# thu-ml/stochastic_gcn

Hardware: AMD Instinct MI355X
Metric: training edges/s (SpMM) (higher is better)
Workload: dtype f32

## Files before the change

stochastic_gcn_amd/csrc/sgcn_dense.hip:

```cpp
#include <algorithm>

#include "sgcn_dev.h"
#include "sgcn_fuse.h"

namespace sgcn {

__device__ __forceinline__ float wave_sum(float v) {
#pragma unroll
    for (int o = 32; o > 0; o >>= 1) v += __shfl_xor(v, o, 64);
    return v;
}
__device__ __forceinline__ float wave_max(float v) {
#pragma unroll
    for (int o = 32; o > 0; o >>= 1) v = fmaxf(v, __shfl_xor(v, o, 64));
    return v;
}

__global__ __launch_bounds__(kBlock) void ln_act_fwd_kernel(
    const float* __restrict__ x, int64_t ldx, const float* __restrict__ offset,
    const float* __restrict__ scale, int32_t n, int32_t d, float eps, int32_t norm, int32_t relu,
    float* __restrict__ y, int64_t ldy, float* __restrict__ xhat, float* __restrict__ rstd) {
    const int lane = threadIdx.x & 63;
    const int64_t row = (int64_t)blockIdx.x * (kBlock / kWave) + threadIdx.x / kWave;
    if (row >= n) return;
// ... 7 lines not shown
    for (int c = lane; c < d; c += kWave) s += xr[c];
    const float mean = wave_sum(s) / (float)d;
    float q = 0.f;
    for (int c = lane; c < d; c += kWave) { const float t = xr[c] - mean; q += t * t; }
    const float r = rsqrtf(wave_sum(q) / (float)d + eps);
    if (lane == 0) rstd[row] = r;
    float* hr = xhat + row * (int64_t)d;
    for (int c = lane; c < d; c += kWave) {
        const float h = (xr[c] - mean) * r;
        hr[c] = h;
        const float v = h * scale[c] + offset[c];
        yr[c] = relu ? fmaxf(v, 0.f) : v;
    }
}

struct LnBwdDx { const float* W; int32_t K, kg; DropArgs drop; float* dxo; int64_t lddxo;
                 int32_t dma; };
struct LnBwdNext { const float* y; int64_t ldy; const float* xhat; const float* rstd; const float* scale; int32_t norm, relu;
                   float* g; float* partial; };

__device__ __forceinline__ void ln_bwd_stats(float g, float h, float sc, float& doff, float& dsc, float& s1, float& s2) {
#pragma clang fp contract(off)
    doff += g;
    dsc = fmaf(g, h, dsc);
    const float t2 = g * sc;
    s1 += t2;
    s2 = fmaf(t2, h, s2);
}
__device__ __forceinline__ float ln_bwd_out(float g, float h, float sc, float m1, float m2, float r) {
#pragma clang fp contract(off)
    return r * fmaf(-h, m2, fmaf(g, sc, -m1));
}

constexpr int kBwdRowsPerWave = 1;
__global__ __launch_bounds__(kBlock) void ln_act_bwd_kernel(
    const float* __restrict__ dy, int64_t lddy, const float* __restrict__ y, int64_t ldy,
    const float* __restrict__ xhat, const float* __restrict__ rstd, const float* __restrict__ scale,
    int32_t n, int32_t d, int32_t norm, int32_t relu, float* __restrict__ dx, int64_t lddx,
    float* __restrict__ partial , LnBwdDx t, LnBwdNext nx) {
    extern __shared__ float lds[];
    const int lane = threadIdx.x & 63, wave = threadIdx.x / kWave;
    const int64_t row0 = ((int64_t)blockIdx.x * (kBlock / kWave) + wave) * kBwdRowsPerWave;
    float* my = lds + (size_t)wave * 2 * d;
    float* wt = lds + (norm ? (size_t)8 * d : 0);
    const int kp = t.K + 1;
    const int wregion = t.dma ? (t.K * d + 255) / 256 * 256 : d * kp;
    if (t.W && t.dma) {
        const int P = d >> 2, sh = __ffs(P) - 1, total4 = t.K * P;
        for (int base4 = wave * kWave; base4 < total4; base4 += kBlock) {
            const int sl = min(base4 + lane, total4 - 1);
            const int j = sl >> sh, src4 = (j << sh) + ((sl & (P - 1)) ^ (j & (P - 1)));
            __builtin_amdgcn_global_load_lds((const __attribute__((address_space(1))) void*)(t.W + (int64_t)src4 * 4),
                                             (__attribute__((address_space(3))) void*)(wt + (int64_t)base4 * 4), 16, 0, 0);
        }
    } else if (t.W) {
        const int total4 = t.K * d / 4;
        const float inv_d = 1.0f / (float)d;
        constexpr int kU = 32;
        float4 v[kU];
        const float4* W4 = reinterpret_cast<const float4*>(t.W);
#pragma unroll
        for (int u = 0; u < kU; u++) { const int i4 = threadIdx.x + u * kBlock; if (i4 < total4) v[u] = W4[i4]; }
#pragma unroll
        for (int u = 0; u < kU; u++) {
            const int i4 = threadIdx.x + u * kBlock;
            if (i4 < total4) {
                const int i = i4 * 4;
                const int j = (int)(((float)i + 0.5f) * inv_d), k = i - j * d;
                float* w = wt + k * kp + j;
                w[0] = v[u].x; w[kp] = v[u].y; w[2 * kp] = v[u].z; w[3 * kp] = v[u].w;
            }
        }
    }
    if (norm) for (int c = lane; c < 2 * d; c += kWave) my[c] = 0.f;
    float gk[2] = {0.f, 0.f};
    bool have = false;
    int64_t myrow = 0;
    for (int k = 0; k < kBwdRowsPerWave; k++) {
        const int64_t row = row0 + k;
        if (row >= n) break;
        have = true; myrow = row;
        const float* gr = dy + row * lddy;
        const float* yr = y + row * ldy;
        float* dr = dx + row * lddx;
        if (!norm) {
            for (int c = lane; c < d; c += kWave) {
                const float g = (relu && !(yr[c] > 0.f)) ? 0.f : gr[c];
                dr[c] = g;
                if (c < 2 * kWave) gk[c / kWave] = g;
            }
            continue;
        }
        const float* hr = xhat + row * (int64_t)d;
        float s1 = 0.f, s2 = 0.f;
        for (int c = lane; c < d; c += kWave) {
            const float g = (relu && !(yr[c] > 0.f)) ? 0.f : gr[c];
            ln_bwd_stats(g, hr[c], scale[c], my[c], my[d + c], s1, s2);
        }
        const float m1 = wave_sum(s1) / (float)d, m2 = wave_sum(s2) / (float)d, r = rstd[row];
        for (int c = lane; c < d; c += kWave) {
            const float g = (relu && !(yr[c] > 0.f)) ? 0.f : gr[c];
            const float o = ln_bwd_out(g, hr[c], scale[c], m1, m2, r);
            dr[c] = o;
            if (c < 2 * kWave) gk[c / kWave] = o;
        }
    }
    if (!norm && !t.W) return;
    if (t.dma) asm volatile("s_waitcnt vmcnt(0)" ::: "memory");
    __syncthreads();
    if (norm) {
        float* out = partial + (size_t)blockIdx.x * 2 * d;
        for (int c = threadIdx.x; c < 2 * d; c += kBlock)
            out[c] = (lds[c] + lds[2 * d + c]) + (lds[4 * d + c] + lds[6 * d + c]);
    }
    if (!t.W || (!have && !nx.y)) return;
    const int d2 = t.K;
    float* my2 = lds + (norm ? (size_t)8 * d : 0) + (size_t)wregion + (size_t)wave * 2 * d2;
    if (nx.y && nx.norm) for (int c = lane; c < 2 * d2; c += kWave) my2[c] = 0.f;
    float dyl[2] = {0.f, 0.f};
    if (have) {
    float acc[4][2];
#pragma unroll
    for (int e = 0; e < 4; e++) { acc[e][0] = 0.f; acc[e][1] = 0.f; }
    int jj[4];
#pragma unroll
    for (int e = 0; e < 4; e++) jj[e] = lane + e * kWave < t.K ? lane + e * kWave : 0;
    int rowf[4], sw[4];
    const int Pm = (d >> 2) - 1;
#pragma unroll
    for (int e = 0; e < 4; e++) { rowf[e] = jj[e] * d; sw[e] = jj[e] & Pm; }
    for (int s0 = 0; s0 * 32 < d; s0++) {
        const int gi = t.kg > 1 ? (s0 & 1) : 0;
        const float xs = s0 < 2 ? gk[0] : gk[1];
        const int kb = s0 * 32, lb = kb & (kWave - 1);
        const int kn = min(32, d - kb);
        const float* wk = wt + kb * kp;
        float p[4];
#pragma unroll
        for (int e = 0; e < 4; e++) p[e] = acc[e][gi];
        if (t.dma) {
#pragma unroll
            for (int q = 0; q < 8; q++) {
                const int c = (kb >> 2) + q;
                float4 w[4];
#pragma unroll
                for (int e = 0; e < 4; e++) w[e] = *reinterpret_cast<const float4*>(wt + rowf[e] + ((c ^ sw[e]) << 2));
#pragma unroll
                for (int u = 0; u < 4; u++) {
                    const float xv = __int_as_float(__builtin_amdgcn_readlane(__float_as_int(xs), lb + q * 4 + u));
#pragma unroll
                    for (int e = 0; e < 4; e++)
                        p[e] = fmaf(xv, u == 0 ? w[e].x : u == 1 ? w[e].y : u == 2 ? w[e].z : w[e].w, p[e]);
                }
            }
        } else if (kn == 32) {
#pragma unroll
            for (int q = 0; q < 4; q++) {
                float w[8][4];
#pragma unroll
                for (int u = 0; u < 8; u++)
#pragma unroll
                    for (int e = 0; e < 4; e++) w[u][e] = wk[(q * 8 + u) * kp + jj[e]];
#pragma unroll
                for (int u = 0; u < 8; u++) {
                    const float xv = __int_as_float(__builtin_amdgcn_readlane(__float_as_int(xs), lb + q * 8 + u));
#pragma unroll
                    for (int e = 0; e < 4; e++) p[e] = fmaf(xv, w[u][e], p[e]);
                }
            }
        } else {
            for (int kk = 0; kk < kn; kk++) {
                const float xv = __int_as_float(__builtin_amdgcn_readlane(__float_as_int(xs), lb + kk));
#pragma unroll
                for (int e = 0; e < 4; e++) p[e] = fmaf(xv, wk[kk * kp + jj[e]], p[e]);
            }
        }
#pragma unroll
        for (int e = 0; e < 4; e++) acc[e][gi] = p[e];
    }
#pragma unroll
    for (int e = 0; e < 4; e++) {
        const int j = lane + e * kWave;
        if (j < t.K) {
            float v = t.kg > 1 ? acc[e][0] + acc[e][1] : acc[e][0];
            if (t.drop.on) v *= drop_factor(t.drop, (int)myrow, j);
            t.dxo[myrow * t.lddxo + j] = v;
            if (e < 2) dyl[e] = v;
        }
    }
    }
    if (!nx.y) return;
    if (have) {
        const float* yr = nx.y + myrow * nx.ldy;
        float* gr = nx.g + myrow * (int64_t)d2;
        if (!nx.norm) {
#pragma unroll
            for (int e = 0; e < 2; e++) {
                const int c = lane + e * kWave;
                if (c < d2) gr[c] = (nx.relu && !(yr[c] > 0.f)) ? 0.f : dyl[e];
            }
        } else {
            const float* hr = nx.xhat + myrow * (int64_t)d2;
            float s1 = 0.f, s2 = 0.f, gg[2] = {0.f, 0.f}, hh[2] = {0.f, 0.f}, sc[2] = {0.f, 0.f};
#pragma unroll
            for (int e = 0; e < 2; e++) {
                const int c = lane + e * kWave;
                if (c < d2) {
                    gg[e] = (nx.relu && !(yr[c] > 0.f)) ? 0.f : dyl[e];
                    hh[e] = hr[c]; sc[e] = nx.scale[c];
                    ln_bwd_stats(gg[e], hh[e], sc[e], my2[c], my2[d2 + c], s1, s2);
                }
            }
            const float m1 = wave_sum(s1) / (float)d2, m2 = wave_sum(s2) / (float)d2, r = nx.rstd[myrow];
#pragma unroll
            for (int e = 0; e < 2; e++) {
                const int c = lane + e * kWave;
                if (c < d2) gr[c] = ln_bwd_out(gg[e], hh[e], sc[e], m1, m2, r);
            }
        }
    }
    if (!nx.norm) return;
    __syncthreads();
    const float* l2 = lds + (norm ? (size_t)8 * d : 0) + (size_t)wregion;
    float* out2 = nx.partial + (size_t)blockIdx.x * 2 * d2;
    for (int c = threadIdx.x; c < 2 * d2; c += kBlock)
        out2[c] = (l2[c] + l2[2 * d2 + c]) + (l2[4 * d2 + c] + l2[6 * d2 + c]);
}

__global__ void ln_param_reduce_kernel(const float* __restrict__ partial, int32_t nblk, int32_t d,
                                       float* __restrict__ doffset, float* __restrict__ dscale) {
    ln_param_reduce_cols32(partial, nblk, d, doffset, dscale, (int)blockIdx.x);
}

struct CeDx { const float* W; int64_t ldw; int32_t K, wflat; float* dx; int64_t lddx; DropArgs drop;
              const float* hx; int64_t ldhx; int32_t kg; DropArgs hdrop; float* zout; int64_t ldzo;
              const float* px; int64_t ldpx; int32_t PK, pS, pkchunk, pkg; const float* PW; DropArgs pdrop;
              const float* poff; const float* psc; float peps; int32_t prelu, pepi;
              float* pY; int64_t ldpy; float* pxhat; float* prstd; };

__host__ __device__ inline int ce_w_region(int K, int c) { return (K * c + 255) / 256 * 256; }

__device__ __forceinline__ void ce_dx_stage(const CeDx& t, int c, float* wl) {
    const int lane = threadIdx.x & 63, wave = threadIdx.x >> 6;
    auto copy = [&](const float* src, int floats, float* dst) {
        const int total4 = floats / 4;
        for (int base4 = wave * kWave; base4 < total4; base4 += (kBlock / kWave) * kWave) {
            const int i4 = min(base4 + lane, total4 - 1);
            __builtin_amdgcn_global_load_lds((const __attribute__((address_space(1))) void*)(src + (int64_t)i4 * 4),
                                             (__attribute__((address_space(3))) void*)(dst + (int64_t)base4 * 4), 16, 0, 0);
        }
    };
    const int total = t.K * c;
    if (t.wflat) copy(t.W, total, wl);
    else
        for (int i = threadIdx.x; i < total; i += kBlock) wl[i] = t.W[(int64_t)(i / c) * t.ldw + (i % c)];
    if (t.PW) copy(t.PW, t.PK * t.K, wl + ce_w_region(t.K, c));
    asm volatile("s_waitcnt vmcnt(0)" ::: "memory");
    __syncthreads();
}
// ... 374 lines not shown

__global__ __launch_bounds__(kBlock) void dropout_kernel(const float* __restrict__ x, int64_t ldx,
                                                         int32_t n, int32_t d, DropArgs a,
                                                         float* __restrict__ out, int64_t ldo) {
    const int64_t total = (int64_t)n * d;
    for (int64_t i = (int64_t)blockIdx.x * kBlock + threadIdx.x; i < total; i += (int64_t)gridDim.x * kBlock) {
        const int row = (int)(i / d), col = (int)(i % d);
        out[row * ldo + col] = x[row * ldx + col] * drop_factor(a, row, col);
    }
}

}

using namespace sgcn;

extern "C" int sgcn_ln_act_fwd_f32(const float* x, int64_t ldx, const float* offset,
                                   const float* scale, int32_t n, int32_t d, float eps,
                                   int32_t relu, float* y, int64_t ldy, float* xhat, float* rstd,
                                   void* stream) {
    SGCN_REQUIRE(n >= 0 && d >= 0, "ln_act_fwd: negative size");
    if (n == 0 || d == 0) return SGCN_OK;
    const int norm = (offset && scale) ? 1 : 0;
    SGCN_REQUIRE(x && y && (!norm || (xhat && rstd)), "ln_act_fwd: null operand");
    const unsigned blocks = (unsigned)((n + 3) / 4);
    hipLaunchKernelGGL(ln_act_fwd_kernel, dim3(blocks), dim3(kBlock), 0, (hipStream_t)stream, x, ldx,
                       offset, scale, n, d, eps, norm, relu, y, ldy, xhat, rstd);
    SGCN_HIP_TRY(hipGetLastError());
    return SGCN_OK;
}

extern "C" int64_t sgcn_ln_act_bwd_ws_floats(int32_t n, int32_t d) {
    const int64_t blocks = ((int64_t)n + 4 * kBwdRowsPerWave - 1) / (4 * kBwdRowsPerWave);
    return blocks * 2 * d;
}

int sgcn::ln_act_bwd_launch(const float* dy, int64_t lddy, const float* y, int64_t ldy, const float* xhat,
                            const float* rstd, const float* scale, int32_t n, int32_t d, int32_t relu,
                            float* dx, int64_t lddx, float* doffset, float* dscale, float* ws,
                            bool reduce_params, int32_t* nblk, hipStream_t st, const float* tail_W, int32_t tail_K,
                            int32_t tail_kg, const sgcn_dropout_t* tail_drop, float* tail_dx, int64_t tail_lddx,
                            const float* nx_y, int64_t nx_ldy, const float* nx_xhat, const float* nx_rstd, const float* nx_scale,
                            int32_t nx_relu, float* nx_g, float* nx_partial) {
    SGCN_REQUIRE(n >= 0 && d >= 0, "ln_act_bwd: negative size");
    if (nblk) *nblk = 0;
    if (n == 0 || d == 0) return SGCN_OK;
    const int norm = scale ? 1 : 0;
    SGCN_REQUIRE(dy && y && dx && (!norm || (xhat && rstd && doffset && dscale && ws)),
                 "ln_act_bwd: null operand");
    SGCN_REQUIRE(!norm || (size_t)d * 8 * sizeof(float) <= 64 * 1024, "ln_act_bwd: d too large for LDS");
    LnBwdDx t{};
    LnBwdNext nx{};
    size_t lds = norm ? (size_t)d * 8 * sizeof(float) : 0;
    if (tail_W) {
        SGCN_REQUIRE(tail_dx && d <= 2 * kWave && d % 4 == 0 && aligned16(tail_W) && tail_K > 0 && tail_K <= 4 * kWave &&
                     tail_lddx >= tail_K && tail_kg >= 1 && tail_kg <= 2, "ln_act_bwd: bad input-gradient tail");
        t.W = tail_W; t.K = tail_K; t.kg = tail_kg; t.drop = drop_args(tail_drop); t.dxo = tail_dx; t.lddxo = tail_lddx;
        SGCN_REQUIRE(!t.drop.on || t.drop.width == tail_K, "ln_act_bwd: dropout width must be the layer's input width");
        t.dma = (d == 32 || d == 64 || d == 128) ? 1 : 0;
        lds += (t.dma ? ((size_t)tail_K * d + 255) / 256 * 256 : (size_t)d * (tail_K + 1)) * sizeof(float);
        if (nx_y) {
            SGCN_REQUIRE(tail_K <= 2 * kWave && nx_g && nx_ldy >= tail_K && (!nx_scale || (nx_xhat && nx_rstd && nx_partial)),
                         "ln_act_bwd: bad chained layer");
            nx.y = nx_y; nx.ldy = nx_ldy; nx.xhat = nx_xhat; nx.rstd = nx_rstd; nx.scale = nx_scale; nx.norm = nx_scale ? 1 : 0;
            nx.relu = nx_relu; nx.g = nx_g; nx.partial = nx_partial;
            if (nx.norm) lds += (size_t)8 * tail_K * sizeof(float);
        }
        SGCN_REQUIRE(lds <= 160 * 1024, "ln_act_bwd: weights too large for LDS");
        static size_t raised = 0;
        if (lds > 64 * 1024 && lds > raised) {
            (void)hipFuncSetAttribute(reinterpret_cast<const void*>(&ln_act_bwd_kernel), hipFuncAttributeMaxDynamicSharedMemorySize, 160 * 1024);
            raised = 160 * 1024;
        }
    }
    const int rows_per_block = 4 * kBwdRowsPerWave;
    const unsigned blocks = (unsigned)((n + rows_per_block - 1) / rows_per_block);
    hipLaunchKernelGGL(ln_act_bwd_kernel, dim3(blocks), dim3(kBlock), lds, st, dy, lddy, y, ldy, xhat, rstd, scale, n, d, norm,
                       relu, dx, lddx, ws, t, nx);
    if (nblk) *nblk = norm ? (int32_t)blocks : 0;
    if (norm && reduce_params)
        hipLaunchKernelGGL(ln_param_reduce_kernel, dim3((2 * d + kLnRedCols - 1) / kLnRedCols), dim3(256), 0, st, ws,
                           (int32_t)blocks, d, doffset, dscale);
    SGCN_HIP_TRY(hipGetLastError());
    return SGCN_OK;
}

extern "C" int sgcn_ln_act_bwd_f32(const float* dy, int64_t lddy, const float* y, int64_t ldy,
                                   const float* xhat, const float* rstd, const float* scale,
                                   int32_t n, int32_t d, int32_t relu, float* dx, int64_t lddx,
                                   float* doffset, float* dscale, float* ws, void* stream) {
    return sgcn::ln_act_bwd_launch(dy, lddy, y, ldy, xhat, rstd, scale, n, d, relu, dx, lddx, doffset, dscale, ws,
                                   true, nullptr, (hipStream_t)stream);
}

namespace sgcn {
int softmax_stats_launch(const float* rowstat, int32_t n, float* stats, void* stream) {
    hipLaunchKernelGGL(softmax_stats_kernel, dim3(1), dim3(kBlock), 0, (hipStream_t)stream, rowstat, n, stats);
    SGCN_HIP_TRY(hipGetLastError());
    return SGCN_OK;
}
int aux_fork(void* stream, void** aux_stream);

namespace {
struct PendingStats { int on = 0, armed = 0, softmax = 0; const float* rowstat = nullptr; int32_t n = 0, c = 0; float* stats = nullptr; };
PendingStats& pending_stats() { static PendingStats p; return p; }
}
void stats_defer(int on) { pending_stats().on = on; }
int stats_flush(void* stream) {
    PendingStats& p = pending_stats();
    if (!p.armed) return SGCN_OK;
    p.armed = 0;
// ... 282 lines not shown
```

stochastic_gcn_amd/csrc/sgcn_dev.h:

```cpp
#pragma once
#include <hip/hip_runtime.h>
#include <cstdint>
#include <type_traits>
#include "sgcn_host.h"
#include "../../include/sgcn.h"

#define SGCN_HIP_TRY(expr)                                                              \
    do {                                                                                \
        hipError_t e__ = (expr);                                                        \
        if (e__ != hipSuccess)                                                          \
            return sgcn::fail(SGCN_ERR_HIP, "%s: %s", #expr, hipGetErrorString(e__));   \
    } while (0)

#define SGCN_REQUIRE(cond, ...)                                       \
    do {                                                              \
        if (!(cond)) return sgcn::fail(SGCN_ERR_INVALID, __VA_ARGS__); \
    } while (0)

namespace sgcn {

constexpr int kWave = 64;
constexpr int kBlock = 256;

template <int VW> struct Vec;
// ... 209 lines not shown
};
struct ReduceMulti {
    ReduceJob j[kMaxGroup];
    const float* ln_partial[kMaxGroup];
    float* doffset[kMaxGroup];
    float* dscale[kMaxGroup];
    int32_t nblk[kMaxGroup], d[kMaxGroup];
    int32_t gfirst[kMaxGroup + 1], lfirst[kMaxGroup + 1];
    int32_t n, ln_accumulate;
};
__device__ __forceinline__ void reduce_multi_body(const ReduceMulti& R, int b, const AdamArgs* adam) {
    if (b < R.gfirst[R.n]) {
        int q = 0;
#pragma unroll
        for (int t = 1; t < kMaxGroup; t++) q += (t < R.n && b >= R.gfirst[t]) ? 1 : 0;
        const ReduceJob& j = R.j[q];
        const int64_t i = (int64_t)(b - R.gfirst[q]) * blockDim.x + threadIdx.x;
        const int64_t mn = (int64_t)j.M * j.N;
        if (i >= mn) return;
        float s = 0.f;
        for (int z = 0; z < j.S; z++) s += j.ws[(int64_t)z * mn + i];
        float* p = j.C + (i / j.N) * j.ldc + (i % j.N);
        const float g = j.accumulate ? *p + s : s;
        *p = g;
        if (adam) adam_one(*adam, p - adam->grad, g);
    } else {
        int q = 0;
#pragma unroll
        for (int t = 1; t < kMaxGroup; t++) q += (t < R.n && b >= R.lfirst[t]) ? 1 : 0;
        ln_param_reduce_cols32(R.ln_partial[q], R.nblk[q], R.d[q], R.doffset[q], R.dscale[q], b - R.lfirst[q], R.ln_accumulate != 0, adam);
    }
}

int ln_act_bwd_launch(const float* dy, int64_t lddy, const float* y, int64_t ldy, const float* xhat,
                      const float* rstd, const float* scale, int32_t n, int32_t d, int32_t relu, float* dx,
                      int64_t lddx, float* doffset, float* dscale, float* ws, bool reduce_params, int32_t* nblk,
                      hipStream_t st, const float* tail_W = nullptr, int32_t tail_K = 0, int32_t tail_kg = 1,
                      const sgcn_dropout_t* tail_drop = nullptr, float* tail_dx = nullptr, int64_t tail_lddx = 0,
                      const float* nx_y = nullptr, int64_t nx_ldy = 0, const float* nx_xhat = nullptr, const float* nx_rstd = nullptr,
                      const float* nx_scale = nullptr, int32_t nx_relu = 0, float* nx_g = nullptr, float* nx_partial = nullptr);

}
```

stochastic_gcn_amd/csrc/sgcn_gemm.hip:

```cpp
#include "sgcn_dev.h"
#include "sgcn_bwd.h"

namespace sgcn {

typedef float f16acc __attribute__((ext_vector_type(16)));

constexpr int kTM = 32, kTN = 128, kTK = 32;

struct GemmArgs {
    const float* A; int64_t lda;
    const float* B; int64_t ldb;
    float* C; int64_t ldc;
    int32_t M, N, K;
    int32_t accumulate;
    int32_t kchunk;
    float* ws;
    const float* offset; const float* scale; float eps; int32_t relu;
    float* xhat; float* rstd;
    int32_t epi;
    const float* A2; int64_t lda2; int32_t a_split;
    DropArgs drop_a;
    DropArgs drop_c;
    int32_t vec_a, vec_b;
    const int32_t* a_gidx;
// ... 787 lines not shown
            c.off += need;
            s.st_dw = c.st;
        }
    }
    return SGCN_OK;
}

static int store_mode_zero(const DenseBwdArgs& a, void* stream) {
    if (!g_grad_store || a.N <= 0 || a.K <= 0) return SGCN_OK;
    hipStream_t st = (hipStream_t)stream;
    if (a.dW) SGCN_HIP_TRY(hipMemset2DAsync(a.dW, (size_t)a.lddw * sizeof(float), 0, (size_t)a.N * sizeof(float), (size_t)a.K, st));
    if (a.doffset) SGCN_HIP_TRY(hipMemsetAsync(a.doffset, 0, (size_t)a.N * sizeof(float), st));
    if (a.dscale) SGCN_HIP_TRY(hipMemsetAsync(a.dscale, 0, (size_t)a.N * sizeof(float), st));
    return SGCN_OK;
}

static int dense_bwd_run(const DenseBwdArgs& a, const BwdScratch& s, void* stream, const DenseBwdArgs* lower = nullptr,
                         const BwdScratch* slower = nullptr, bool* lower_done = nullptr, int32_t* lower_nblk = nullptr) {
    SGCN_REQUIRE(a.n >= 0 && a.N >= 0 && a.K >= 0, "dense_bwd: negative size");
    if (a.n == 0 || a.N == 0 || a.K == 0) return store_mode_zero(a, stream);
    SGCN_REQUIRE(a.dy && a.x && a.W && a.dW, "dense_bwd: null operand");
    hipStream_t st = (hipStream_t)stream;
    const float* g = a.dy;
    int64_t ldg = a.lddy;
    int32_t nblk = 0;
    bool dx_in_row_pass = false;
    int dx_kg = 1;
    if (lower_done && !lower && *lower_done) {
        nblk = lower_nblk ? *lower_nblk : 0;
        g = a.g_tmp; ldg = a.N;
    } else if (a.scale || a.relu) {
        SGCN_REQUIRE(a.g_tmp && a.y, "dense_bwd: LayerNorm / ReLU backward needs y and an n x N scratch");
        SGCN_REQUIRE(!a.scale || a.ws, "dense_bwd: LayerNorm backward needs the workspace");
        if (a.dx && (tune_get("step_fuse") & 8) && a.N <= 128 && a.N % 4 == 0 && a.K <= 256 && a.ldw == a.N && aligned16(a.W) &&
            (size_t)(8 * a.N + a.N * (a.K + 1)) * sizeof(float) <= 160 * 1024) {
            int S = 0, kgq = 0;
            const sgcn_dropout_t* dr = a.drop;
            if (dr && dr->keep >= 1.0f) dr = nullptr;
            if (dr) { S = 1; GemmArgs q{}; q.M = a.n; q.N = a.K; q.K = a.N; kgq = prepare_gemm(q, nullptr).kgroups; }
            else gemm_fwd_shape(a.n, a.K, a.N, &S, &kgq, nullptr);
            if (S == 1 && kgq <= 2) dx_in_row_pass = true, dx_kg = kgq;
        }
        const bool chain = dx_in_row_pass && lower && slower && lower_done && a.K <= 128 && lower->dy == a.dx && lower->lddy == a.lddx &&
                           lower->n == a.n && lower->N == a.K && (lower->scale || lower->relu) && lower->g_tmp && lower->y &&
                           (!lower->scale || (lower->xhat && lower->rstd && slower->ws_ln)) &&
                           (size_t)(8 * a.N + a.N * (a.K + 1) + 8 * a.K) * sizeof(float) <= 160 * 1024;
        const int rc = ln_act_bwd_launch(a.dy, a.lddy, a.y, a.ldy, a.xhat, a.rstd, a.scale, a.n, a.N, a.relu, a.g_tmp, a.N,
                                         a.doffset, a.dscale, s.ws_ln, false, &nblk, st,
                                         dx_in_row_pass ? a.W : nullptr, a.K, dx_kg, a.drop, a.dx, a.lddx,
                                         chain ? lower->y : nullptr, chain ? lower->ldy : 0, chain ? lower->xhat : nullptr,
                                         chain ? lower->rstd : nullptr, chain ? lower->scale : nullptr, chain ? lower->relu : 0,
                                         chain ? lower->g_tmp : nullptr, chain ? slower->ws_ln : nullptr);
        if (rc != SGCN_OK) return rc;
        if (chain) {
            *lower_done = true;
            if (lower_nblk) *lower_nblk = (lower->scale && a.scale) ? nblk : (lower->scale ? (a.n + 3) / 4 : 0);
        }
        g = a.g_tmp; ldg = a.N;
    }
    if (s.st_dw != st) {
        AuxCtx& c = aux_ctx();
        SGCN_HIP_TRY(hipEventRecord(c.fork, st));
        SGCN_HIP_TRY(hipStreamWaitEvent(c.st, c.fork, 0));
        c.pending = true;
    }
    GemmArgs q{};
    q.A = a.x; q.lda = a.ldx; q.B = g; q.ldb = ldg; q.C = a.dW; q.ldc = a.lddw;
    q.M = a.K; q.N = a.N; q.K = a.n; q.accumulate = g_grad_store ? 0 : 1; q.epi = 0;
    q.a_gidx = a.gidx;
    q.drop_a = drop_args(a.drop);
    SGCN_REQUIRE(!q.drop_a.on || q.drop_a.width == a.K, "dense_bwd: dropout width must be K");
    ReduceJob job{};
    int rc = SGCN_OK;
    if (s.deferred) {
        DwGroupState& dg = dw_state();
        DwJob& J = dg.jobs[dg.n++];
// ... 75 lines not shown
```

stochastic_gcn_amd/csrc/sgcn_spmm.hip:

```cpp
#include "sgcn_dev.h"
#include <cstring>

namespace sgcn {

namespace {
int g_tune_nv = 0;
int g_tune_unroll = 0;
int g_tune_slabmajor = 1;
int g_tune_cs_round = 0;
int g_tune_cs_unroll = 0;
int g_tune_cs_pace = 0;
int g_tune_cs_slack = 0;
int g_tune_cs_noextra = 0;
int g_tune_step_overlap = 1;
int g_tune_step_fuse = 127;
int g_tune_cs_g2_wide = 0;
int g_tune_cs_nowarp = 0;
int g_tune_cs_last_pct = 80;
int g_tune_gemm_min_steps = 0;
int g_tune_gemm_mb16_slice_k = 0;
int g_tune_lds_wave_bias = 100;
int g_tune_lds_mix = 1;
int g_tune_lds_dbg = 0;
thread_local int tl_step_overlap = -1, tl_step_fuse = -1;
}

void step_mode_override(int overlap, int fuse) { tl_step_overlap = overlap; tl_step_fuse = fuse; }

int tune_get(const char* key) {
    if (!strcmp(key, "spmm_nv")) return g_tune_nv;
    if (!strcmp(key, "spmm_unroll")) return g_tune_unroll;
    if (!strcmp(key, "spmm_slabmajor")) return g_tune_slabmajor;
    if (!strcmp(key, "cs_round")) return g_tune_cs_round;
    if (!strcmp(key, "cs_unroll")) return g_tune_cs_unroll;
    if (!strcmp(key, "cs_pace")) return g_tune_cs_pace;
    if (!strcmp(key, "cs_slack")) return g_tune_cs_slack;
    if (!strcmp(key, "cs_noextra")) return g_tune_cs_noextra;
    if (!strcmp(key, "step_overlap")) return tl_step_overlap >= 0 ? tl_step_overlap : g_tune_step_overlap;
    if (!strcmp(key, "step_fuse")) return tl_step_fuse >= 0 ? tl_step_fuse : g_tune_step_fuse;
    if (!strcmp(key, "cs_g2_wide")) return g_tune_cs_g2_wide;
    if (!strcmp(key, "cs_nowarp")) return g_tune_cs_nowarp;
    if (!strcmp(key, "cs_last_pct")) return g_tune_cs_last_pct;
    if (!strcmp(key, "gemm_min_steps")) return g_tune_gemm_min_steps;
    if (!strcmp(key, "gemm_mb16_slice_k")) return g_tune_gemm_mb16_slice_k;
    if (!strcmp(key, "lds_wave_bias")) return g_tune_lds_wave_bias;
    if (!strcmp(key, "lds_mix")) return g_tune_lds_mix;
    if (!strcmp(key, "lds_dbg")) return g_tune_lds_dbg;
    return -1;
}

struct SpmmArgs {
    const int32_t* rowptr;
    const int32_t* col;
    const float* val;
    const sgcn_seg_t* seg;
    int64_t nseg;
    int64_t nsegblk;
    const void* B;
    int64_t ldb;
    const int32_t* gidx;
    const float* rscale;
    const float* cscale;
    float* C;
    int64_t ldc;
    float beta;
    int32_t d;
    int32_t nvec;
    float* ws;
    int64_t ldw;
    int32_t slabmajor;
    const float* add;
    int64_t ldadd;
    int32_t add_rows;
};

template <int VW>
__device__ __forceinline__ void epilogue_store(const SpmmArgs& a, int row, int vi,
                                               typename Vec<VW>::type acc, float rs) {
    float* out = a.C + (int64_t)row * a.ldc + (int64_t)vi * VW;
    typename Vec<VW>::type r = acc * rs;
// ... 174 lines not shown
    if (nvec <= 32) return 32;
    return 64;
}

}

using namespace sgcn;

extern "C" int64_t sgcn_tune_get(const char* key) { return key ? tune_get(key) : -1; }

extern "C" int sgcn_tune(const char* key, int64_t value) {
    if (!key) return fail(SGCN_ERR_INVALID, "sgcn_tune: null key");
    if (!strcmp(key, "spmm_nv")) { SGCN_REQUIRE(value >= 0 && value <= 4, "spmm_nv in 0..4"); g_tune_nv = (int)value; return SGCN_OK; }
    if (!strcmp(key, "spmm_unroll")) {
        SGCN_REQUIRE(value == 0 || value == 2 || value == 4 || value == 8, "spmm_unroll in {0,2,4,8}");
        g_tune_unroll = (int)value; return SGCN_OK;
    }
    if (!strcmp(key, "spmm_slabmajor")) { g_tune_slabmajor = value != 0; return SGCN_OK; }
    if (!strcmp(key, "cs_pace")) { SGCN_REQUIRE(value >= 0, "cs_pace >= 0"); g_tune_cs_pace = (int)value; return SGCN_OK; }
    if (!strcmp(key, "cs_slack")) { SGCN_REQUIRE(value >= 0, "cs_slack >= 0"); g_tune_cs_slack = (int)value; return SGCN_OK; }
    if (!strcmp(key, "cs_noextra")) { g_tune_cs_noextra = value != 0; return SGCN_OK; }
    if (!strcmp(key, "step_overlap")) { g_tune_step_overlap = value != 0; return SGCN_OK; }
    if (!strcmp(key, "step_fuse")) { SGCN_REQUIRE(value >= 0 && value <= 127, "step_fuse in 0..127"); g_tune_step_fuse = (int)value; return SGCN_OK; }
    if (!strcmp(key, "cs_g2_wide")) { g_tune_cs_g2_wide = value != 0; return SGCN_OK; }
    if (!strcmp(key, "cs_nowarp")) { g_tune_cs_nowarp = value != 0; return SGCN_OK; }
    if (!strcmp(key, "gemm_min_steps")) { g_tune_gemm_min_steps = (int)value; return SGCN_OK; }
    if (!strcmp(key, "gemm_mb16_slice_k")) {
        SGCN_REQUIRE(value >= 0 && value <= 0x7fffffff, "gemm_mb16_slice_k >= 0");
        g_tune_gemm_mb16_slice_k = (int)value; return SGCN_OK;
    }
    if (!strcmp(key, "lds_wave_bias")) { SGCN_REQUIRE(value >= 50 && value <= 300, "lds_wave_bias in 50..300 (per cent)"); g_tune_lds_wave_bias = (int)value; return SGCN_OK; }
    if (!strcmp(key, "lds_mix")) { g_tune_lds_mix = value != 0; return SGCN_OK; }
    if (!strcmp(key, "lds_dbg")) { g_tune_lds_dbg = (int)value; return SGCN_OK; }
    if (!strcmp(key, "cs_last_pct")) { SGCN_REQUIRE(value >= 0 && value <= 100, "cs_last_pct in [0, 100]"); g_tune_cs_last_pct = (int)value; return SGCN_OK; }
    if (!strcmp(key, "cs_round")) { SGCN_REQUIRE(value >= 0, "cs_round >= 0"); g_tune_cs_round = (int)value; return SGCN_OK; }
    if (!strcmp(key, "cs_unroll")) {
        SGCN_REQUIRE(value == 0 || value == 4 || value == 8, "cs_unroll in {0,4,8}");
        g_tune_cs_unroll = (int)value; return SGCN_OK;
    }
    return fail(SGCN_ERR_INVALID, "sgcn_tune: unknown key '%s'", key);
}

template <class BT>
static int spmm_csr_add(const int32_t* rowptr, const int32_t* col, const float* val,
                        int32_t M, int32_t K, int32_t d, const BT* B, int64_t ldb,
                        const int32_t* gidx, const float* rscale, const float* cscale,
                        float* C, int64_t ldc, float beta, const sgcn_plan_t* plan,
                        const float* add, int64_t ldadd, int32_t add_rows, void* stream) {
    constexpr bool kB16 = !std::is_same<BT, float>::value;
    SGCN_REQUIRE(M >= 0 && K >= 0 && d >= 0, "spmm: negative size");
    if (M == 0 || d == 0) return SGCN_OK;
    SGCN_REQUIRE(rowptr && C && (B || K == 0), "spmm: null operand");
    SGCN_REQUIRE(ldb >= d && ldc >= d, "spmm: leading dimension smaller than d");
    if (kB16) {
        SGCN_REQUIRE(ldb % 8 == 0, "spmm: a bfloat16 operand needs ldb %% 8 == 0 (ldb %lld, d %d)", (long long)ldb, d);
        SGCN_REQUIRE(aligned16(B), "spmm: a bfloat16 operand needs a 16-byte aligned base");
    }
    hipStream_t st = (hipStream_t)stream;

    SpmmArgs a{};
    a.rowptr = rowptr; a.col = col; a.val = val;
    a.B = B; a.ldb = ldb; a.gidx = gidx; a.rscale = rscale; a.cscale = cscale;
    a.C = C; a.ldc = ldc; a.beta = beta; a.d = d;
    a.nseg = M;
    a.slabmajor = g_tune_slabmajor;
    if (add && add_rows > 0) {
// ... 86 lines not shown
```

Before: 7.415 billion.

## Add persistent grid-stride LayerNorm backward kernel for large row counts

Adds a streaming LN/activation backward kernel that launches a capped number of blocks, each walking rows with a grid stride. For d<=128 it keeps scale and the per-column parameter-gradient accumulators in registers. It is enabled by default when n exceeds 16384 rows. This shrinks the per-block partial workspace and the cost of the parameter reduction, and stages W once per block instead of once per four rows. In exchange it disables the chained fused path and, unless the tail knob is set, the in-row-pass dx fusion for large n, which could add separate GEMM passes.

New measurement: 7.418 billion (median of 6 runs). About the same (+0.1%).

```diff
diff --git a/profiles/ln_bwd_stream_probe.py b/profiles/ln_bwd_stream_probe.py
--- /dev/null
+++ b/profiles/ln_bwd_stream_probe.py
@@ -0,0 +1,81 @@
+#!/usr/bin/env python
+import argparse
+import json
+import os
+import sys
+
+ROOT = os.path.dirname(os.path.dirname(os.path.abspath(__file__)))
+sys.path.insert(0, ROOT)
+
+MODES = (("one_row", -1, 0), ("stream_tail", 8, 1), ("stream_mfma", 8, -1))
+
+
+def _timed(fn, reps, warm=3):
+    import torch
+    for _ in range(warm):
+        fn()
+    e0, e1 = torch.cuda.Event(enable_timing=True), torch.cuda.Event(enable_timing=True)
+    torch.cuda.synchronize()
+    e0.record()
+    for _ in range(reps):
+        fn()
+    e1.record()
+    e1.synchronize()
+    return e0.elapsed_time(e1) * 1e3 / reps
+
+
+def main():
+    ap = argparse.ArgumentParser()
+    ap.add_argument("--reps", type=int, default=20)
+    ap.add_argument("--rows", default="1024,2048,4096,8192,16384,32768,65536,131072,232965")
+    args = ap.parse_args()
+    import torch
+    from stochastic_gcn_amd import _ffi, ops
+    dev = torch.device("cuda:0")
+    ops.pin_stream()
+    d = 128
+    g = torch.Generator(device="cpu").manual_seed(1)
+    for n in [int(v) for v in args.rows.split(",")]:
+        dy = torch.randn((n, d), generator=g).to(dev)
+        pre = torch.randn((n, d), generator=g).to(dev)
+        off = (0.1 * torch.randn((1, d), generator=g)).to(dev)
+        scl = (1 + 0.1 * torch.randn((1, d), generator=g)).to(dev)
+        y, ctx = ops.ln_act_fwd(pre, off, scl, True)
+        rec = {"what": "ln_bwd_stream", "n": n, "d": d, "reps": args.reps}
+        try:
+            for name, rows, tail in MODES[:2]:
+                _ffi.tune("ln_bwd_stream_rows", rows)
+                doff, dsc = torch.zeros((1, d), device=dev), torch.zeros((1, d), device=dev)
+                rec["ln_act_bwd_%s_us" % name.split("_tail")[0]] = _timed(
+                    lambda: ops.ln_act_bwd(dy, y, ctx, scl, True, doff, dsc), args.reps)
+            for K in (128, 256):
+                x = torch.randn((n, K), generator=g).to(dev)
+                W = (torch.randn((K, d), generator=g) / K ** 0.5).to(dev)
+                drop = ops.Drop(0.8, 77)
+                outs = {}
+                for name, rows, tail in MODES:
+                    _ffi.tune("ln_bwd_stream_rows", rows)
+                    _ffi.tune("ln_bwd_stream_tail", tail)
+
+                    def call():
+                        dW = torch.zeros((K, d), device=dev)
+                        doff, dsc = torch.zeros((1, d), device=dev), torch.zeros((1, d), device=dev)
+                        return ops.dense_bwd(dy, y, ctx, scl, True, x, W, dW, doff, dsc, need_dx=True, drop=drop), dW, doff, dsc
+                    rec["dense_bwd_K%d_%s_us" % (K, name)] = _timed(call, args.reps)
+                    outs[name] = call()
+                torch.cuda.synchronize()
+                rec["K%d_dx_bits_equal" % K] = all(torch.equal(outs["one_row"][0], outs[m][0]) for m in ("stream_tail", "stream_mfma"))
+                rec["K%d_dW_bits_equal" % K] = all(torch.equal(outs["one_row"][1], outs[m][1]) for m in ("stream_tail", "stream_mfma"))
+                rec["K%d_stream_forms_param_bits_equal" % K] = bool(
+                    torch.equal(outs["stream_tail"][2], outs["stream_mfma"][2]) and torch.equal(outs["stream_tail"][3], outs["stream_mfma"][3]))
+                del x, outs
+        finally:
+            _ffi.tune("ln_bwd_stream_rows", 0)
+            _ffi.tune("ln_bwd_stream_tail", 0)
+        print(json.dumps(rec), flush=True)
+        del dy, pre, y, ctx
+        torch.cuda.empty_cache()
+
+
+if __name__ == "__main__":
+    main()
diff --git a/stochastic_gcn_amd/csrc/sgcn_dense.hip b/stochastic_gcn_amd/csrc/sgcn_dense.hip
--- a/stochastic_gcn_amd/csrc/sgcn_dense.hip
+++ b/stochastic_gcn_amd/csrc/sgcn_dense.hip
@@ -63,6 +63,174 @@
     return r * fmaf(-h, m2, fmaf(g, sc, -m1));
 }
 
+__device__ __forceinline__ void ln_bwd_stage(const LnBwdDx& t, int d, float* wt, int kp, int lane, int wave) {
+    if (t.W && t.dma) {
+        const int P = d >> 2, sh = __ffs(P) - 1, total4 = t.K * P;
+        for (int base4 = wave * kWave; base4 < total4; base4 += kBlock) {
+            const int sl = min(base4 + lane, total4 - 1);
+            const int j = sl >> sh, src4 = (j << sh) + ((sl & (P - 1)) ^ (j & (P - 1)));
+            __builtin_amdgcn_global_load_lds((const __attribute__((address_space(1))) void*)(t.W + (int64_t)src4 * 4),
+                                             (__attribute__((address_space(3))) void*)(wt + (int64_t)base4 * 4), 16, 0, 0);
+        }
+    } else if (t.W) {
+        const int total4 = t.K * d / 4;
+        const float inv_d = 1.0f / (float)d;
+        constexpr int kU = 32;
+        float4 v[kU];
+        const float4* W4 = reinterpret_cast<const float4*>(t.W);
+#pragma unroll
+        for (int u = 0; u < kU; u++) { const int i4 = threadIdx.x + u * kBlock; if (i4 < total4) v[u] = W4[i4]; }
+#pragma unroll
+        for (int u = 0; u < kU; u++) {
+            const int i4 = threadIdx.x + u * kBlock;
+            if (i4 < total4) {
+                const int i = i4 * 4;
+                const int j = (int)(((float)i + 0.5f) * inv_d), k = i - j * d;
+                float* w = wt + k * kp + j;
+                w[0] = v[u].x; w[kp] = v[u].y; w[2 * kp] = v[u].z; w[3 * kp] = v[u].w;
+            }
+        }
+    }
+}
+
+__device__ __forceinline__ void ln_bwd_row(const float* __restrict__ dy, int64_t lddy, const float* __restrict__ y, int64_t ldy,
+                                           const float* __restrict__ xhat, const float* __restrict__ rstd,
+                                           const float* __restrict__ scale, int32_t d, int32_t norm, int32_t relu,
+                                           float* __restrict__ dx, int64_t lddx, int64_t row, int lane, float* my, float gk[2]) {
+    const float* gr = dy + row * lddy;
+    const float* yr = y + row * ldy;
+    float* dr = dx + row * lddx;
+    if (!norm) {
+        for (int c = lane; c < d; c += kWave) {
+            const float g = (relu && !(yr[c] > 0.f)) ? 0.f : gr[c];
+            dr[c] = g;
+            if (c < 2 * kWave) gk[c / kWave] = g;
+        }
+        return;
+    }
+    const float* hr = xhat + row * (int64_t)d;
+    float s1 = 0.f, s2 = 0.f;
+    for (int c = lane; c < d; c += kWave) {
+        const float g = (relu && !(yr[c] > 0.f)) ? 0.f : gr[c];
+        ln_bwd_stats(g, hr[c], scale[c], my[c], my[d + c], s1, s2);
+    }
+    const float m1 = wave_sum(s1) / (float)d, m2 = wave_sum(s2) / (float)d, r = rstd[row];
+    for (int c = lane; c < d; c += kWave) {
+        const float g = (relu && !(yr[c] > 0.f)) ? 0.f : gr[c];
+        const float o = ln_bwd_out(g, hr[c], scale[c], m1, m2, r);
+        dr[c] = o;
+        if (c < 2 * kWave) gk[c / kWave] = o;
+    }
+}
+
+__device__ __forceinline__ void ln_bwd_row_regs(const float* __restrict__ dy, int64_t lddy, const float* __restrict__ y, int64_t ldy,
+                                                const float* __restrict__ xhat, const float* __restrict__ rstd, const float sc[2],
+                                                int32_t d, int32_t norm, int32_t relu, float* __restrict__ dx, int64_t lddx,
+                                                int64_t row, int lane, float cs[4], float gk[2]) {
+    const float* gr = dy + row * lddy;
+    const float* yr = y + row * ldy;
+    const float* hr = xhat + row * (int64_t)d;
+    float* dr = dx + row * lddx;
+    float g[2] = {0.f, 0.f}, h[2] = {0.f, 0.f};
+    const float r = norm ? rstd[row] : 0.f;
+#pragma unroll
+    for (int e = 0; e < 2; e++) {
+        const int c = lane + e * kWave;
+        if (c < d) {
+            g[e] = (relu && !(yr[c] > 0.f)) ? 0.f : gr[c];
+            if (norm) h[e] = hr[c];
+        }
+    }
+    if (norm) {
+        float s1 = 0.f, s2 = 0.f;
+#pragma unroll
+        for (int e = 0; e < 2; e++)
+            if (lane + e * kWave < d) ln_bwd_stats(g[e], h[e], sc[e], cs[e], cs[2 + e], s1, s2);
+        const float m1 = wave_sum(s1) / (float)d, m2 = wave_sum(s2) / (float)d;
+#pragma unroll
+        for (int e = 0; e < 2; e++) g[e] = ln_bwd_out(g[e], h[e], sc[e], m1, m2, r);
+    }
+#pragma unroll
+    for (int e = 0; e < 2; e++) {
+        const int c = lane + e * kWave;
+        if (c < d) dr[c] = g[e];
+        gk[e] = c < d ? g[e] : 0.f;
+    }
+}
+
+__device__ __forceinline__ void ln_bwd_tail_row(const LnBwdDx& t, int d, const float* wt, int kp, const float gk[2],
+                                                int64_t myrow, int lane, float dyl[2]) {
+    float acc[4][2];
+#pragma unroll
+    for (int e = 0; e < 4; e++) { acc[e][0] = 0.f; acc[e][1] = 0.f; }
+    int jj[4];
+#pragma unroll
+    for (int e = 0; e < 4; e++) jj[e] = lane + e * kWave < t.K ? lane + e * kWave : 0;
+    int rowf[4], sw[4];
+    const int Pm = (d >> 2) - 1;
+#pragma unroll
+    for (int e = 0; e < 4; e++) { rowf[e] = jj[e] * d; sw[e] = jj[e] & Pm; }
+    for (int s0 = 0; s0 * 32 < d; s0++) {
+        const int gi = t.kg > 1 ? (s0 & 1) : 0;
+        const float xs = s0 < 2 ? gk[0] : gk[1];
+        const int kb = s0 * 32, lb = kb & (kWave - 1);
+        const int kn = min(32, d - kb);
+        const float* wk = wt + kb * kp;
+        float p[4];
+#pragma unroll
+        for (int e = 0; e < 4; e++) p[e] = acc[e][gi];
+        if (t.dma) {
+#pragma unroll
+            for (int q = 0; q < 8; q++) {
+                const int c = (kb >> 2) + q;
+                float4 w[4];
+#pragma unroll
+                for (int e = 0; e < 4; e++) w[e] = *reinterpret_cast<const float4*>(wt + rowf[e] + ((c ^ sw[e]) << 2));
+#pragma unroll
+                for (int u = 0; u < 4; u++) {
+                    const float xv = __int_as_float(__builtin_amdgcn_readlane(__float_as_int(xs), lb + q * 4 + u));
+#pragma unroll
+                    for (int e = 0; e < 4; e++)
+                        p[e] = fmaf(xv, u == 0 ? w[e].x : u == 1 ? w[e].y : u == 2 ? w[e].z : w[e].w, p[e]);
+                }
+            }
+        } else if (kn == 32) {
+#pragma unroll
+            for (int q = 0; q < 4; q++) {
+                float w[8][4];
+#pragma unroll
+                for (int u = 0; u < 8; u++)
+#pragma unroll
+                    for (int e = 0; e < 4; e++) w[u][e] = wk[(q * 8 + u) * kp + jj[e]];
+#pragma unroll
+                for (int u = 0; u < 8; u++) {
+                    const float xv = __int_as_float(__builtin_amdgcn_readlane(__float_as_int(xs), lb + q * 8 + u));
+#pragma unroll
+                    for (int e = 0; e < 4; e++) p[e] = fmaf(xv, w[u][e], p[e]);
+                }
+            }
+        } else {
+            for (int kk = 0; kk < kn; kk++) {
+                const float xv = __int_as_float(__builtin_amdgcn_readlane(__float_as_int(xs), lb + kk));
+#pragma unroll
+                for (int e = 0; e < 4; e++) p[e] = fmaf(xv, wk[kk * kp + jj[e]], p[e]);
+            }
+        }
+#pragma unroll
+        for (int e = 0; e < 4; e++) acc[e][gi] = p[e];
+    }
+#pragma unroll
+    for (int e = 0; e < 4; e++) {
+        const int j = lane + e * kWave;
+        if (j < t.K) {
+            float v = t.kg > 1 ? acc[e][0] + acc[e][1] : acc[e][0];
+            if (t.drop.on) v *= drop_factor(t.drop, (int)myrow, j);
+            t.dxo[myrow * t.lddxo + j] = v;
+            if (e < 2) dyl[e] = v;
+        }
+    }
+}
+
 constexpr int kBwdRowsPerWave = 1;
 __global__ __launch_bounds__(kBlock) void ln_act_bwd_kernel(
     const float* __restrict__ dy, int64_t lddy, const float* __restrict__ y, int64_t ldy,
@@ -76,33 +244,7 @@
     float* wt = lds + (norm ? (size_t)8 * d : 0);
     const int kp = t.K + 1;
     const int wregion = t.dma ? (t.K * d + 255) / 256 * 256 : d * kp;
-    if (t.W && t.dma) {
-        const int P = d >> 2, sh = __ffs(P) - 1, total4 = t.K * P;
-        for (int base4 = wave * kWave; base4 < total4; base4 += kBlock) {
-            const int sl = min(base4 + lane, total4 - 1);
-            const int j = sl >> sh, src4 = (j << sh) + ((sl & (P - 1)) ^ (j & (P - 1)));
-            __builtin_amdgcn_global_load_lds((const __attribute__((address_space(1))) void*)(t.W + (int64_t)src4 * 4),
-                                             (__attribute__((address_space(3))) void*)(wt + (int64_t)base4 * 4), 16, 0, 0);
-        }
-    } else if (t.W) {
-        const int total4 = t.K * d / 4;
-        const float inv_d = 1.0f / (float)d;
-        constexpr int kU = 32;
-        float4 v[kU];
-        const float4* W4 = reinterpret_cast<const float4*>(t.W);
-#pragma unroll
-        for (int u = 0; u < kU; u++) { const int i4 = threadIdx.x + u * kBlock; if (i4 < total4) v[u] = W4[i4]; }
-#pragma unroll
-        for (int u = 0; u < kU; u++) {
-            const int i4 = threadIdx.x + u * kBlock;
-            if (i4 < total4) {
-                const int i = i4 * 4;
-                const int j = (int)(((float)i + 0.5f) * inv_d), k = i - j * d;
-                float* w = wt + k * kp + j;
-                w[0] = v[u].x; w[kp] = v[u].y; w[2 * kp] = v[u].z; w[3 * kp] = v[u].w;
-            }
-        }
-    }
+    ln_bwd_stage(t, d, wt, kp, lane, wave);
     if (norm) for (int c = lane; c < 2 * d; c += kWave) my[c] = 0.f;
     float gk[2] = {0.f, 0.f};
     bool have = false;
@@ -111,30 +253,7 @@
         const int64_t row = row0 + k;
         if (row >= n) break;
         have = true; myrow = row;
-        const float* gr = dy + row * lddy;
-        const float* yr = y + row * ldy;
-        float* dr = dx + row * lddx;
-        if (!norm) {
-            for (int c = lane; c < d; c += kWave) {
-                const float g = (relu && !(yr[c] > 0.f)) ? 0.f : gr[c];
-                dr[c] = g;
-                if (c < 2 * kWave) gk[c / kWave] = g;
-            }
-            continue;
-        }
-        const float* hr = xhat + row * (int64_t)d;
-        float s1 = 0.f, s2 = 0.f;
-        for (int c = lane; c < d; c += kWave) {
-            const float g = (relu && !(yr[c] > 0.f)) ? 0.f : gr[c];
-            ln_bwd_stats(g, hr[c], scale[c], my[c], my[d + c], s1, s2);
-        }
-        const float m1 = wave_sum(s1) / (float)d, m2 = wave_sum(s2) / (float)d, r = rstd[row];
-        for (int c = lane; c < d; c += kWave) {
-            const float g = (relu && !(yr[c] > 0.f)) ? 0.f : gr[c];
-            const float o = ln_bwd_out(g, hr[c], scale[c], m1, m2, r);
-            dr[c] = o;
-            if (c < 2 * kWave) gk[c / kWave] = o;
-        }
+        ln_bwd_row(dy, lddy, y, ldy, xhat, rstd, scale, d, norm, relu, dx, lddx, row, lane, my, gk);
     }
     if (!norm && !t.W) return;
     if (t.dma) asm volatile("s_waitcnt vmcnt(0)" ::: "memory");
@@ -149,77 +268,7 @@
     float* my2 = lds + (norm ? (size_t)8 * d : 0) + (size_t)wregion + (size_t)wave * 2 * d2;
     if (nx.y && nx.norm) for (int c = lane; c < 2 * d2; c += kWave) my2[c] = 0.f;
     float dyl[2] = {0.f, 0.f};
-    if (have) {
-    float acc[4][2];
-#pragma unroll
-    for (int e = 0; e < 4; e++) { acc[e][0] = 0.f; acc[e][1] = 0.f; }
-    int jj[4];
-#pragma unroll
-    for (int e = 0; e < 4; e++) jj[e] = lane + e * kWave < t.K ? lane + e * kWave : 0;
-    int rowf[4], sw[4];
-    const int Pm = (d >> 2) - 1;
-#pragma unroll
-    for (int e = 0; e < 4; e++) { rowf[e] = jj[e] * d; sw[e] = jj[e] & Pm; }
-    for (int s0 = 0; s0 * 32 < d; s0++) {
-        const int gi = t.kg > 1 ? (s0 & 1) : 0;
-        const float xs = s0 < 2 ? gk[0] : gk[1];
-        const int kb = s0 * 32, lb = kb & (kWave - 1);
-        const int kn = min(32, d - kb);
-        const float* wk = wt + kb * kp;
-        float p[4];
-#pragma unroll
-        for (int e = 0; e < 4; e++) p[e] = acc[e][gi];
-        if (t.dma) {
-#pragma unroll
-            for (int q = 0; q < 8; q++) {
-                const int c = (kb >> 2) + q;
-                float4 w[4];
-#pragma unroll
-                for (int e = 0; e < 4; e++) w[e] = *reinterpret_cast<const float4*>(wt + rowf[e] + ((c ^ sw[e]) << 2));
-#pragma unroll
-                for (int u = 0; u < 4; u++) {
-                    const float xv = __int_as_float(__builtin_amdgcn_readlane(__float_as_int(xs), lb + q * 4 + u));
-#pragma unroll
-                    for (int e = 0; e < 4; e++)
-                        p[e] = fmaf(xv, u == 0 ? w[e].x : u == 1 ? w[e].y : u == 2 ? w[e].z : w[e].w, p[e]);
-                }
-            }
-        } else if (kn == 32) {
-#pragma unroll
-            for (int q = 0; q < 4; q++) {
-                float w[8][4];
-#pragma unroll
-                for (int u = 0; u < 8; u++)
-#pragma unroll
-                    for (int e = 0; e < 4; e++) w[u][e] = wk[(q * 8 + u) * kp + jj[e]];
-#pragma unroll
-                for (int u = 0; u < 8; u++) {
-                    const float xv = __int_as_float(__builtin_amdgcn_readlane(__float_as_int(xs), lb + q * 8 + u));
-#pragma unroll
-                    for (int e = 0; e < 4; e++) p[e] = fmaf(xv, w[u][e], p[e]);
-                }
-            }
-        } else {
-            for (int kk = 0; kk < kn; kk++) {
-                const float xv = __int_as_float(__builtin_amdgcn_readlane(__float_as_int(xs), lb + kk));
-#pragma unroll
-                for (int e = 0; e < 4; e++) p[e] = fmaf(xv, wk[kk * kp + jj[e]], p[e]);
-            }
-        }
-#pragma unroll
-        for (int e = 0; e < 4; e++) acc[e][gi] = p[e];
-    }
-#pragma unroll
-    for (int e = 0; e < 4; e++) {
-        const int j = lane + e * kWave;
-        if (j < t.K) {
-            float v = t.kg > 1 ? acc[e][0] + acc[e][1] : acc[e][0];
-            if (t.drop.on) v *= drop_factor(t.drop, (int)myrow, j);
-            t.dxo[myrow * t.lddxo + j] = v;
-            if (e < 2) dyl[e] = v;
-        }
-    }
-    }
+    if (have) ln_bwd_tail_row(t, d, wt, kp, gk, myrow, lane, dyl);
     if (!nx.y) return;
     if (have) {
         const float* yr = nx.y + myrow * nx.ldy;
@@ -256,6 +305,55 @@
     float* out2 = nx.partial + (size_t)blockIdx.x * 2 * d2;
     for (int c = threadIdx.x; c < 2 * d2; c += kBlock)
         out2[c] = (l2[c] + l2[2 * d2 + c]) + (l2[4 * d2 + c] + l2[6 * d2 + c]);
+}
+
+constexpr int kLnStreamBlocks = 1024;
+template <bool kTail>
+__global__ __launch_bounds__(kBlock) void ln_act_bwd_stream_kernel(
+    const float* __restrict__ dy, int64_t lddy, const float* __restrict__ y, int64_t ldy,
+    const float* __restrict__ xhat, const float* __restrict__ rstd, const float* __restrict__ scale,
+    int32_t n, int32_t d, int32_t norm, int32_t relu, float* __restrict__ dx, int64_t lddx,
+    float* __restrict__ partial , LnBwdDx t) {
+    extern __shared__ float lds[];
+    const int lane = threadIdx.x & 63, wave = threadIdx.x / kWave;
+    float* my = lds + (size_t)wave * 2 * d;
+    float* wt = lds + (norm ? (size_t)8 * d : 0);
+    const int kp = t.K + 1;
+    if (kTail) ln_bwd_stage(t, d, wt, kp, lane, wave);
+    if (norm) for (int c = lane; c < 2 * d; c += kWave) my[c] = 0.f;
+    if (kTail) {
+        if (t.dma) asm volatile("s_waitcnt vmcnt(0)" ::: "memory");
+        __syncthreads();
+    }
+    const int64_t stride = (int64_t)gridDim.x * (kBlock / kWave);
+    const int64_t first = (int64_t)blockIdx.x * (kBlock / kWave) + wave;
+    if (d <= 2 * kWave) {
+        float cs[4] = {0.f, 0.f, 0.f, 0.f}, sc[2] = {0.f, 0.f};
+        if (norm) {
+            if (lane < d) sc[0] = scale[lane];
+            if (lane + kWave < d) sc[1] = scale[lane + kWave];
+        }
+        for (int64_t row = first; row < n; row += stride) {
+            float gk[2], dyl[2];
+            ln_bwd_row_regs(dy, lddy, y, ldy, xhat, rstd, sc, d, norm, relu, dx, lddx, row, lane, cs, gk);
+            if (kTail) ln_bwd_tail_row(t, d, wt, kp, gk, row, lane, dyl);
+        }
+        if (norm) {
+            if (lane < d) { my[lane] = cs[0]; my[d + lane] = cs[2]; }
+            if (lane + kWave < d) { my[lane + kWave] = cs[1]; my[d + lane + kWave] = cs[3]; }
+        }
+    } else {
+        for (int64_t row = first; row < n; row += stride) {
+            float gk[2] = {0.f, 0.f}, dyl[2];
+            ln_bwd_row(dy, lddy, y, ldy, xhat, rstd, scale, d, norm, relu, dx, lddx, row, lane, my, gk);
+            if (kTail) ln_bwd_tail_row(t, d, wt, kp, gk, row, lane, dyl);
+        }
+    }
+    if (!norm) return;
+    __syncthreads();
+    float* out = partial + (size_t)blockIdx.x * 2 * d;
+    for (int c = threadIdx.x; c < 2 * d; c += kBlock)
+        out[c] = (lds[c] + lds[2 * d + c]) + (lds[4 * d + c] + lds[6 * d + c]);
 }
 
 __global__ void ln_param_reduce_kernel(const float* __restrict__ partial, int32_t nblk, int32_t d,
@@ -696,6 +794,12 @@
 extern "C" int64_t sgcn_ln_act_bwd_ws_floats(int32_t n, int32_t d) {
     const int64_t blocks = ((int64_t)n + 4 * kBwdRowsPerWave - 1) / (4 * kBwdRowsPerWave);
     return blocks * 2 * d;
+}
+
+constexpr int32_t kLnStreamRowsDefault = 16384;
+bool sgcn::ln_bwd_streams(int32_t n) {
+    const int knob = tune_get("ln_bwd_stream_rows");
+    return knob >= 0 && n > (knob > 0 ? knob : kLnStreamRowsDefault);
 }
 
 int sgcn::ln_act_bwd_launch(const float* dy, int64_t lddy, const float* y, int64_t ldy, const float* xhat,
@@ -737,9 +841,24 @@
         }
     }
     const int rows_per_block = 4 * kBwdRowsPerWave;
-    const unsigned blocks = (unsigned)((n + rows_per_block - 1) / rows_per_block);
-    hipLaunchKernelGGL(ln_act_bwd_kernel, dim3(blocks), dim3(kBlock), lds, st, dy, lddy, y, ldy, xhat, rstd, scale, n, d, norm,
-                       relu, dx, lddx, ws, t, nx);
+    unsigned blocks = (unsigned)((n + rows_per_block - 1) / rows_per_block);
+    if (!nx.y && ln_bwd_streams(n)) {
+        blocks = (unsigned)std::min<int64_t>(kLnStreamBlocks, ((int64_t)n + 3) / 4);
+        static size_t raised_stream = 0;
+        if (lds > 64 * 1024 && lds > raised_stream) {
+            (void)hipFuncSetAttribute(reinterpret_cast<const void*>(&ln_act_bwd_stream_kernel<true>), hipFuncAttributeMaxDynamicSharedMemorySize, 160 * 1024);
+            raised_stream = 160 * 1024;
+        }
+        if (t.W)
+            hipLaunchKernelGGL(ln_act_bwd_stream_kernel<true>, dim3(blocks), dim3(kBlock), lds, st, dy, lddy, y, ldy, xhat, rstd, scale,
+                               n, d, norm, relu, dx, lddx, ws, t);
+        else
+            hipLaunchKernelGGL(ln_act_bwd_stream_kernel<false>, dim3(blocks), dim3(kBlock), lds, st, dy, lddy, y, ldy, xhat, rstd, scale,
+                               n, d, norm, relu, dx, lddx, ws, t);
+    } else {
+        hipLaunchKernelGGL(ln_act_bwd_kernel, dim3(blocks), dim3(kBlock), lds, st, dy, lddy, y, ldy, xhat, rstd, scale, n, d, norm,
+                           relu, dx, lddx, ws, t, nx);
+    }
     if (nblk) *nblk = norm ? (int32_t)blocks : 0;
     if (norm && reduce_params)
         hipLaunchKernelGGL(ln_param_reduce_kernel, dim3((2 * d + kLnRedCols - 1) / kLnRedCols), dim3(256), 0, st, ws,
diff --git a/stochastic_gcn_amd/csrc/sgcn_dev.h b/stochastic_gcn_amd/csrc/sgcn_dev.h
--- a/stochastic_gcn_amd/csrc/sgcn_dev.h
+++ b/stochastic_gcn_amd/csrc/sgcn_dev.h
@@ -265,6 +265,7 @@
     }
 }
 
+bool ln_bwd_streams(int32_t n);
 int ln_act_bwd_launch(const float* dy, int64_t lddy, const float* y, int64_t ldy, const float* xhat,
                       const float* rstd, const float* scale, int32_t n, int32_t d, int32_t relu, float* dx,
                       int64_t lddx, float* doffset, float* dscale, float* ws, bool reduce_params, int32_t* nblk,
diff --git a/stochastic_gcn_amd/csrc/sgcn_gemm.hip b/stochastic_gcn_amd/csrc/sgcn_gemm.hip
--- a/stochastic_gcn_amd/csrc/sgcn_gemm.hip
+++ b/stochastic_gcn_amd/csrc/sgcn_gemm.hip
@@ -843,7 +843,8 @@
     } else if (a.scale || a.relu) {
         SGCN_REQUIRE(a.g_tmp && a.y, "dense_bwd: LayerNorm / ReLU backward needs y and an n x N scratch");
         SGCN_REQUIRE(!a.scale || a.ws, "dense_bwd: LayerNorm backward needs the workspace");
-        if (a.dx && (tune_get("step_fuse") & 8) && a.N <= 128 && a.N % 4 == 0 && a.K <= 256 && a.ldw == a.N && aligned16(a.W) &&
+        const bool stream_tail = tune_get("ln_bwd_stream_tail") > 0;
+        if (a.dx && (tune_get("step_fuse") & 8) && (stream_tail || !ln_bwd_streams(a.n)) && a.N <= 128 && a.N % 4 == 0 && a.K <= 256 && a.ldw == a.N && aligned16(a.W) &&
             (size_t)(8 * a.N + a.N * (a.K + 1)) * sizeof(float) <= 160 * 1024) {
             int S = 0, kgq = 0;
             const sgcn_dropout_t* dr = a.drop;
@@ -852,7 +853,7 @@
             else gemm_fwd_shape(a.n, a.K, a.N, &S, &kgq, nullptr);
             if (S == 1 && kgq <= 2) dx_in_row_pass = true, dx_kg = kgq;
         }
-        const bool chain = dx_in_row_pass && lower && slower && lower_done && a.K <= 128 && lower->dy == a.dx && lower->lddy == a.lddx &&
+        const bool chain = !ln_bwd_streams(a.n) && dx_in_row_pass && lower && slower && lower_done && a.K <= 128 && lower->dy == a.dx && lower->lddy == a.lddx &&
                            lower->n == a.n && lower->N == a.K && (lower->scale || lower->relu) && lower->g_tmp && lower->y &&
                            (!lower->scale || (lower->xhat && lower->rstd && slower->ws_ln)) &&
                            (size_t)(8 * a.N + a.N * (a.K + 1) + 8 * a.K) * sizeof(float) <= 160 * 1024;
diff --git a/stochastic_gcn_amd/csrc/sgcn_spmm.hip b/stochastic_gcn_amd/csrc/sgcn_spmm.hip
--- a/stochastic_gcn_amd/csrc/sgcn_spmm.hip
+++ b/stochastic_gcn_amd/csrc/sgcn_spmm.hip
@@ -21,6 +21,8 @@
 int g_tune_gemm_mb16_slice_k = 0;
 int g_tune_lds_wave_bias = 100;
 int g_tune_lds_mix = 1;
+int g_tune_ln_bwd_stream_rows = 0;
+int g_tune_ln_bwd_stream_tail = 0;
 int g_tune_lds_dbg = 0;
 thread_local int tl_step_overlap = -1, tl_step_fuse = -1;
 }
@@ -46,6 +48,8 @@
     if (!strcmp(key, "lds_wave_bias")) return g_tune_lds_wave_bias;
     if (!strcmp(key, "lds_mix")) return g_tune_lds_mix;
     if (!strcmp(key, "lds_dbg")) return g_tune_lds_dbg;
+    if (!strcmp(key, "ln_bwd_stream_rows")) return g_tune_ln_bwd_stream_rows;
+    if (!strcmp(key, "ln_bwd_stream_tail")) return g_tune_ln_bwd_stream_tail;
     return -1;
 }
 
@@ -286,6 +290,11 @@
     if (!strcmp(key, "lds_wave_bias")) { SGCN_REQUIRE(value >= 50 && value <= 300, "lds_wave_bias in 50..300 (per cent)"); g_tune_lds_wave_bias = (int)value; return SGCN_OK; }
     if (!strcmp(key, "lds_mix")) { g_tune_lds_mix = value != 0; return SGCN_OK; }
     if (!strcmp(key, "lds_dbg")) { g_tune_lds_dbg = (int)value; return SGCN_OK; }
+    if (!strcmp(key, "ln_bwd_stream_rows")) {
+        SGCN_REQUIRE(value <= 0x7fffffff, "ln_bwd_stream_rows < 2^31 (0: the default, negative: never)");
+        g_tune_ln_bwd_stream_rows = value < 0 ? -1 : (int)value; return SGCN_OK;
+    }
+    if (!strcmp(key, "ln_bwd_stream_tail")) { g_tune_ln_bwd_stream_tail = value < 0 ? -1 : value > 0 ? 1 : 0; return SGCN_OK; }
     if (!strcmp(key, "cs_last_pct")) { SGCN_REQUIRE(value >= 0 && value <= 100, "cs_last_pct in [0, 100]"); g_tune_cs_last_pct = (int)value; return SGCN_OK; }
     if (!strcmp(key, "cs_round")) { SGCN_REQUIRE(value >= 0, "cs_round >= 0"); g_tune_cs_round = (int)value; return SGCN_OK; }
     if (!strcmp(key, "cs_unroll")) {
```
